# Mehran-Memon/fspann-query-system

Hardware: AMD Instinct MI355X
Metric: queries/sec @ recall@10, SIFT-1M-shaped synthetic data d=128 B=256 (higher is better)
Workload: dtype f64

## Files before the change

fspann-query-system_amd/csrc/route_lazy.hip.h:

```cpp
#pragma once
#include "route.hip.h"

namespace fspann {

constexpr uint64_t kLzEmpty = ~0ull;
constexpr int kLzThreads = 256;
constexpr int kLzEntriesMax = 1024;
constexpr int kLzCollMax = 256;
constexpr int lz_ht_size(int kEnt) { return 2 * kEnt; }
constexpr int lz_sort_max(int kEnt) { return kEnt - 128; }
constexpr size_t lz_order_bytes(int TP) {
    return static_cast<size_t>(TP + 2) * 8 + ((static_cast<size_t>(TP + 1) * 4 + 7) & ~size_t(7)) + static_cast<size_t>(TP) * 8 +
           ((static_cast<size_t>(TP) * 2 + 3) & ~size_t(3));
}
constexpr size_t lz_lds_bytes(int kEnt, int TD, int P) {
    const size_t tp = static_cast<size_t>(TD) * P, ord_gk = lz_order_bytes(TD * P), gk = static_cast<size_t>(lz_sort_max(kEnt)) * 4;
    return static_cast<size_t>(lz_ht_size(kEnt)) * 8 + tp * 16 + static_cast<size_t>(kEnt) * 4 + 4096 +
           (((ord_gk > gk ? ord_gk : gk) + 7) & ~size_t(7)) + static_cast<size_t>(TD) * 8 + static_cast<size_t>(kEnt) * 2 +
           static_cast<size_t>(lz_sort_max(kEnt)) * 2 * 2 + static_cast<size_t>(TD) * 4 +
           (kEnt != 512 ? static_cast<size_t>(TD) * 4 + tp * 4 : 0);
}
static_assert(lz_lds_bytes(512, 16, 5) == 20152 && lz_lds_bytes(512, 16, 5) + 256 <= 160 * 1024 / 8, "eight per CU at 16 x 5");
constexpr int lz_stage_u(int) { return 4; }
constexpr int lz_keep(int) { return 8; }

#ifdef FSPANN_DEBUG_STAMPS
__device__ __forceinline__ long long dbg_hw_where() {
    uint32_t hw, xcc;
    asm volatile("s_getreg_b32 %0, hwreg(HW_REG_HW_ID)" : "=s"(hw));
    asm volatile("s_getreg_b32 %0, hwreg(HW_REG_XCC_ID)" : "=s"(xcc));
    return (static_cast<long long>(xcc) << 32) | hw;
}
#endif

__device__ __forceinline__ int wave_cut1024(const int32_t* bins, int need, int lane, int* before) {
    const int4* b4 = reinterpret_cast<const int4*>(bins) + lane * 4;
    const int4 v0 = b4[0], v1 = b4[1], v2 = b4[2], v3 = b4[3];
    const int vals[16] = {v0.x, v0.y, v0.z, v0.w, v1.x, v1.y, v1.z, v1.w, v2.x, v2.y, v2.z, v2.w, v3.x, v3.y, v3.z, v3.w};
    int sum = 0;
#pragma unroll
    for (int i = 0; i < 16; i++) sum += vals[i];
    int incl = sum;
#pragma unroll
    for (int off = 1; off < 64; off <<= 1) {
        const int v = __shfl_up(incl, off);
        if (lane >= off) incl += v;
    }
    const int excl = incl - sum;
    const unsigned long long bm = __ballot((incl >= need) && (excl < need));
    if (bm == 0) {
        *before = __shfl(incl, 63) - __shfl(v3.w, 63);
        return 1023;
    }
    const int src = __ffsll(static_cast<long long>(bm)) - 1;
    int cum = excl, bb = 15;
    bool found = false;
#pragma unroll
    for (int i = 0; i < 16; i++) {
        if (!found) {
            if (cum + vals[i] >= need) { bb = i; found = true; }
            else cum += vals[i];
        }
    }
    *before = __shfl(cum, src);
    return __shfl(lane * 16 + bb, src);
}

template <int kThreads, int kEnt = kLzEntriesMax, bool kChk = true, int kTD = 0, int kP = 0, bool kList = false>
__device__ __forceinline__ void route_lazy_run(const RouteParams& prm, unsigned char* smem, const int64_t q_first, const int64_t q_stride, const int block_id) {
    int4* probe_in = prm.probe_g;
    int32_t* nprobe_in = prm.nprobe_g;
    int tid = threadIdx.x;
    constexpr int nthreads = kThreads;
    constexpr int nwv = kThreads / 64;
    int lane = tid & 63, wave = __builtin_amdgcn_readfirstlane(tid >> 6);
    const int TD = kTD > 0 ? kTD : prm.TD, P = kP > 0 ? kP : prm.P, S = (kTD > 0) ? 64 : prm.S;
    const int TP = TD * P;
    const int SP = (S + 63) >> 6;

    constexpr int kLzHtSize = lz_ht_size(kEnt), kLzEntries = kEnt, kLzSortMax = lz_sort_max(kEnt);
    constexpr int kLzStageU = lz_stage_u(kEnt), kLzKeep = lz_keep(kEnt);
    static_assert(kEnt == 512 || kEnt == 1024 || kEnt == 2048, "size classes");
    static_assert(!(kChk && kEnt == 512), "the 512-entry class has no registers for the check");
    size_t o = 0;
    uint64_t* ht = reinterpret_cast<uint64_t*>(smem + o);        o += static_cast<size_t>(kLzHtSize) * 8;
    int4* plist = reinterpret_cast<int4*>(smem + o);             o += static_cast<size_t>(TP) * 16;
    uint32_t* pre = reinterpret_cast<uint32_t*>(smem + o);       o += static_cast<size_t>(kEnt) * 4;
    int32_t* bins = reinterpret_cast<int32_t*>(smem + o);        o += 1024 * 4;
    const size_t o_ord = o;
    uint2* pkv = reinterpret_cast<uint2*>(smem + o);             o += (static_cast<size_t>(TP) + 2) * 8;
    int32_t* pcs = reinterpret_cast<int32_t*>(smem + o);         o += (static_cast<size_t>(TP) + 1) * 4;
    o = (o + 7) & ~size_t(7);
    int64_t* pbase = reinterpret_cast<int64_t*>(smem + o);       o += static_cast<size_t>(TP) * 8;
    uint16_t* ord = reinterpret_cast<uint16_t*>(smem + o);
    uint32_t* gk = reinterpret_cast<uint32_t*>(smem + o_ord);
    o = o_ord + ((max(lz_order_bytes(TP), static_cast<size_t>(kLzSortMax) * 4) + 7) & ~size_t(7));
    int64_t* ids_base = reinterpret_cast<int64_t*>(smem + o);    o += static_cast<size_t>(TD) * 8;
    uint16_t* ulist = reinterpret_cast<uint16_t*>(smem + o);     o += static_cast<size_t>(kLzEntries) * 2;
    uint16_t* rk = reinterpret_cast<uint16_t*>(smem + o);        o += static_cast<size_t>(kLzSortMax) * 2;
    uint16_t* lrank = reinterpret_cast<uint16_t*>(smem + o);     o += static_cast<size_t>(kLzSortMax) * 2;
    int32_t* nprobe_l = reinterpret_cast<int32_t*>(smem + o);    o += static_cast<size_t>(TD) * 4;
    int32_t* part0 = reinterpret_cast<int32_t*>(smem + o);       if (kEnt != 512) o += static_cast<size_t>(TD) * 4;
    int32_t* pglob = reinterpret_cast<int32_t*>(smem + o);
    int32_t* c_elem = bins;
    int32_t* c_lt = bins + kLzCollMax;
    int32_t* c_id = bins + 2 * kLzCollMax;
    int32_t* c_seq = bins + 3 * kLzCollMax;

    __shared__ int s_u, s_R, s_ncoll, s_bad, s_b, s_cnt, s_short, s_susp;
    constexpr uint32_t ht_mask = kLzHtSize - 1;
    constexpr int ht_shift = (kEnt == 2048) ? 32 - 12 : (kEnt == 1024) ? 32 - 11 : 32 - 10;
    unsigned long long lt_mask = 0;

    for (int i = tid; i < TD; i += nthreads) { ids_base[i] = prm.tables[i].ids_base; if (kChk) part0[i] = static_cast<int32_t>(prm.tables[i].part_base); }
    for (int i = tid; i < kLzHtSize; i += nthreads) ht[i] = kLzEmpty;
    if (kChk && prm.bin16) for (int i = tid; i < 1024; i += nthreads) bins[i] = 0;
    if (block_id == 0 && tid == 0) *prm.ovf_next = 0;
    __syncthreads();

    auto present = [&](int32_t id) -> bool {
        uint32_t slot = (static_cast<uint32_t>(id) * 2654435761u) >> ht_shift;
        const uint32_t stp = ((static_cast<uint32_t>(id) * 0x85EBCA6Bu) >> ht_shift) | 1u;
        for (int tries = 0; tries < kLzHtSize; tries++) {
            const uint64_t e = ht[slot];
            if (e == kLzEmpty) return false;
            if (static_cast<uint32_t>(e >> 32) == static_cast<uint32_t>(id)) return true;
            slot = (slot + stp) & ht_mask;
        }
        return false;
    };
    auto insert = [&](int32_t id, uint32_t low, uint32_t* slot_out) -> bool {
        const uint64_t mine = (static_cast<uint64_t>(static_cast<uint32_t>(id)) << 32) | low;
        uint32_t slot = (static_cast<uint32_t>(id) * 2654435761u) >> ht_shift;
        const uint32_t stp = ((static_cast<uint32_t>(id) * 0x85EBCA6Bu) >> ht_shift) | 1u;
        for (int tries = 0; tries < kLzHtSize; tries++) {
            const uint64_t old = atomicCAS(reinterpret_cast<unsigned long long*>(&ht[slot]), kLzEmpty, mine);
            if (old == kLzEmpty) { *slot_out = slot; return true; }
            if (static_cast<uint32_t>(old >> 32) == static_cast<uint32_t>(id)) {
                if (static_cast<uint32_t>(old) > low) atomicMin(reinterpret_cast<unsigned long long*>(&ht[slot]), mine);
                return false;
            }
            slot = (slot + stp) & ht_mask;
        }
        s_bad = 1;
        return false;
    };

#ifdef FSPANN_DEBUG_STAMPS
#define LZ_STAMP(i) do { if (prm.dbg && tid == 0 && qi == block_id) prm.dbg[block_id * 16 + (i)] = wall_clock64(); } while (0)
#else
#define LZ_STAMP(i) do { } while (0)
#endif
#ifdef FSPANN_LZ_STOP_AFTER
#define LZ_STOP(n) if (FSPANN_LZ_STOP_AFTER == (n) && prm.nq > 0) { __syncthreads(); if (tid == 0) prm.out_count[qi] = 0;               \
        const int used_ = min(s_u, kLzEntries); for (int i_ = tid; i_ < used_; i_ += nthreads) ht[ulist[i_]] = kLzEmpty; __syncthreads(); continue; }
#else
#define LZ_STOP(n)
#endif
#define LZ_FOR_TUPLES(RA, RB, BODY)                                                                                   \
    do {                                                                                                              \
        const int nit_ = ((RB) - (RA)) * SP;                                                                          \
        for (int it0_ = wave; it0_ < nit_; it0_ += nwv * kLzStageU) {                                                 \
            uint64_t entv_[kLzStageU];                                                                                \
            int scv_[kLzStageU];                                                                                      \
            _Pragma("unroll") for (int v_ = 0; v_ < kLzStageU; v_++) {                                                \
                const int it_ = it0_ + v_ * nwv;                                                                      \
                entv_[v_] = kLzEmpty; scv_[v_] = 0;                                                                   \
                if (it_ < nit_) {                                                                                     \
                    const int rr_ = (RA) + it_ / SP, pos_ = (it_ % SP) * 64 + lane;                                   \
                    const int pi_ = ord[rr_];                                                                         \
                    const int4 pr_ = plist[pi_];                                                                      \
                    scv_[v_] = pr_.y;                                                                                 \
                    if (pos_ < pr_.w) entv_[v_] = prm.ids_bk[pbase[pi_] + pos_];                                      \
                }                                                                                                     \
            }                                                                                                         \
            _Pragma("unroll") for (int v_ = 0; v_ < kLzStageU; v_++) {                                                \
                if (it0_ + v_ * nwv >= nit_) continue;                                                                \
                int32_t id = static_cast<int32_t>(entv_[v_] >> 32);                              \
                const uint32_t bf = static_cast<uint32_t>(entv_[v_]); (void)bf;                                       \
                const int sc = scv_[v_]; (void)sc;                                                                    \
                if (id >= 0 && prm.deleted_bits && ((prm.deleted_bits[id >> 5] >> (id & 31)) & 1u)) id = -1;  \
                BODY                                                                                                  \
            }                                                                                                         \
        }                                                                                                             \
    } while (0)
#define LZ_INSERT(COND, LOW)                                                                                          \
    do {                                                                                                              \
        bool created_ = false;                                                                                        \
        uint32_t slot_ = 0;                                                                                           \
        if (COND) created_ = insert(id, (LOW), &slot_);                                                               \
        const unsigned long long bm_ = __ballot(created_);                                                            \
        if (bm_) {                                                                                                    \
            int base_ = 0;                                                                                            \
            if (lane == 0) base_ = atomicAdd(&s_u, __popcll(bm_));                                                    \
            base_ = __shfl(base_, 0);                                                                                 \
            const int at_ = base_ + __popcll(bm_ & lt_mask);                                                          \
            if (created_ && at_ < kLzEntries) ulist[at_] = static_cast<uint16_t>(slot_);                              \
        }                                                                                                             \
    } while (0)

    const int64_t nq_eff = kList ? static_cast<int64_t>(*prm.qcount) : prm.nq;
    for (int64_t qs = q_first; qs < nq_eff; qs += q_stride) {
        const int64_t qi = kList ? static_cast<int64_t>(prm.qlist[qs]) : qs;
        LZ_STAMP(0);
        if (prm.probe_G > 0) {
            const int G = (kTD > 0) ? 16 : prm.probe_G, lgG = 31 - __clz(G), ngroups = nthreads >> lgG;
            const int grp_in_wave = lane >> lgG, gl = lane & (G - 1), grp = tid >> lgG;
            int32_t* w3 = reinterpret_cast<int32_t*>(pre) + grp * (2 * P - 1) * 3;
            for (int t0 = 0; t0 < TD; t0 += ngroups) {
                const int td = t0 + grp;
                const bool act = td < TD;
                const int tdc = act ? td : 0;
                const int Wc = (kTD > 0) ? 1 : prm.W;
#ifdef FSPANN_DEBUG_STAMPS
                long long* pst = (prm.dbg && tid == 0 && qi == block_id && t0 == 0) ? prm.dbg + (static_cast<long long>(gridDim.x) + block_id) * 16 : nullptr;
#else
                long long* pst = nullptr;
#endif
                const int np = route_probe_table<int4*, kP, (kTD > 0 ? 1 : 0)>(prm, act, prm.codes + (qi * TD + tdc) * Wc, prm.tables[tdc], G, gl, grp_in_wave,
                                                                             w3, plist + tdc * P, pst);
                if (act && gl == 0) nprobe_l[td] = np;
            }
            __syncthreads();
            for (int i = tid; i < TP; i += nthreads) {
                const int td = i / P, step = i - td * P;
                int4 e = make_int4(-1, 0x7FFF, 0, 0);
                if (step < nprobe_l[td]) e = plist[i];
                plist[i] = e;
                pbase[i] = ids_base[td] + e.z;
                if (kChk) pglob[i] = part0[td] + e.x;
                pkv[i] = make_uint2((static_cast<uint32_t>(e.y) << 16) | static_cast<uint32_t>(i), static_cast<uint32_t>(e.w));
            }
        } else {
            for (int i = tid; i < TP; i += nthreads) {
                const int td = i / P, step = i - td * P;
                int4 e = make_int4(-1, 0x7FFF, 0, 0);
                if (step < nprobe_in[qi * TD + td]) e = probe_in[qi * TP + i];
                plist[i] = e;
                pbase[i] = ids_base[td] + e.z;
                if (kChk) pglob[i] = part0[td] + e.x;
                pkv[i] = make_uint2((static_cast<uint32_t>(e.y) << 16) | static_cast<uint32_t>(i), static_cast<uint32_t>(e.w));
            }
        }
        if (tid == 0) {
            s_u = 0; s_R = TP; s_ncoll = 0; s_bad = 0; s_short = 0; s_susp = 0;
            if (TP & 1) pkv[TP] = make_uint2(0xFFFFFFFFu, 0u);
        }
        __syncthreads();
        LZ_STAMP(1);
        LZ_STOP(1)
        asm volatile("" : "+v"(tid));
        lane = tid & 63; wave = __builtin_amdgcn_readfirstlane(tid >> 6);
        lt_mask = (1ull << lane) - 1ull;
        constexpr int kChkU = 5;
        uint2 chk_v[kChkU];
        int chk_n[kChkU];
        const int chk_cps = prm.bin16_shift - 2;
        const int chk_items = (kChk && prm.bin16) ? (TP << chk_cps) : 0;
        const bool chk_once = chk_items <= nthreads * kChkU;
        auto chk_load = [&](const int it0) {
#pragma unroll
            for (int v = 0; v < kChkU; v++) {
                const int it = it0 + v * nthreads;
                chk_v[v] = make_uint2(0u, 0u); chk_n[v] = 0;
                if (it < chk_items) {
                    const int pi = it >> chk_cps, ch = it & ((1 << chk_cps) - 1);
                    const int4 pr = plist[pi];
                    const int rem = pr.w - ch * 4;
                    if (pr.x >= 0 && rem > 0) {
                        chk_v[v] = *reinterpret_cast<const uint2*>(prm.bin16 + (static_cast<int64_t>(pglob[pi]) << prm.bin16_shift) + ch * 4);
                        chk_n[v] = min(rem, 4);
                    }
                }
            }
        };
        auto chk_count = [&]() {
            bool sus = false;
#pragma unroll
            for (int v = 0; v < kChkU; v++) {
#pragma unroll
                for (int k = 0; k < 4; k++) {
                    if (k < chk_n[v]) {
                        const uint32_t b16 = ((k < 2 ? chk_v[v].x : chk_v[v].y) >> ((k & 1) * 16)) & 0xFFFFu;
                        const uint32_t sh = (b16 & 7u) * 4u;
                        const uint32_t old = atomicAdd(reinterpret_cast<uint32_t*>(bins) + ((b16 & 8191u) >> 3), 1u << sh);
                        sus = sus || (((old >> sh) & 15u) >= 8u);
                    }
                }
            }
            if (sus) s_susp = 1;
        };
        if (chk_items > 0 && chk_once) chk_load(tid);
        for (int i = tid; i < TP; i += nthreads) {
            const uint2 me = pkv[i];
            const uint32_t mk = me.x;
            int rank = 0, cum = 0;
            const uint4* kv4 = reinterpret_cast<const uint4*>(pkv);
#pragma unroll 4
            for (int j = 0; j < (TP + 1) / 2; j++) {
                const uint4 kv = kv4[j];
                const bool b0 = kv.x < mk, b1 = kv.z < mk;
                rank += b0 + b1;
                cum += (b0 ? kv.y : 0u) + (b1 ? kv.w : 0u);
            }
            ord[rank] = static_cast<uint16_t>(i);
            pcs[rank] = cum;
            if ((mk >> 16) == 0x7FFFu) atomicMin(&s_R, rank);
            if (rank == TP - 1) pcs[TP] = cum + static_cast<int>(me.y);
        }
        if (chk_items > 0) {
            if (chk_once) chk_count();
            else for (int it0 = tid; it0 < chk_items; it0 += nthreads * kChkU) { chk_load(it0); chk_count(); }
        }
        __syncthreads();
        LZ_STAMP(2);
        LZ_STOP(2)
        const int R = s_R;
        bool overflow = false;
        if (chk_items > 0 && s_susp) {
            uint32_t* mark = reinterpret_cast<uint32_t*>(ht);
            uint64_t* cl = ht + 128;
            uint64_t* cf = cl + 256;
            constexpr int kChkList = 256;
            static_assert(128 + 2 * 256 <= lz_ht_size(512), "the check's scratch fits the smallest hash table");
            for (int i = tid; i < 256; i += nthreads) mark[i] = 0u;
            for (int i = tid; i < 1024; i += nthreads) bins[i] = 0;
            __syncthreads();
            for (int it = tid; it < chk_items; it += nthreads) {
                const int pi = it >> chk_cps, ch = it & ((1 << chk_cps) - 1);
                const int4 pr = plist[pi];
                const int rem = pr.w - ch * 4;
                if (pr.x < 0 || rem <= 0) continue;
                const uint2 vv = *reinterpret_cast<const uint2*>(prm.bin16 + (static_cast<int64_t>(pglob[pi]) << prm.bin16_shift) + ch * 4);
                for (int k = 0; k < min(rem, 4); k++) {
                    const uint32_t b16 = ((k < 2 ? vv.x : vv.y) >> ((k & 1) * 16)) & 0xFFFFu, f = b16 & 8191u;
                    const uint32_t sh = (f & 7u) * 4u;
                    const uint32_t old = atomicAdd(reinterpret_cast<uint32_t*>(bins) + (f >> 3), 1u << sh);
                    if (((old >> sh) & 15u) >= 8u) atomicOr(&mark[f >> 5], 1u << (f & 31u));
                }
            }
            __syncthreads();
            for (int it = tid; it < chk_items; it += nthreads) {
                const int pi = it >> chk_cps, ch = it & ((1 << chk_cps) - 1);
                const int4 pr = plist[pi];
                const int rem = pr.w - ch * 4;
                if (pr.x < 0 || rem <= 0) continue;
                const uint2 vv = *reinterpret_cast<const uint2*>(prm.bin16 + (static_cast<int64_t>(pglob[pi]) << prm.bin16_shift) + ch * 4);
                for (int k = 0; k < min(rem, 4); k++) {
                    const uint32_t b16 = ((k < 2 ? vv.x : vv.y) >> ((k & 1) * 16)) & 0xFFFFu, f = b16 & 8191u;
                    if (!((mark[f >> 5] >> (f & 31u)) & 1u)) continue;
                    const int32_t id = prm.ids[pbase[pi] + ch * 4 + k];
                    if (prm.deleted_bits && ((prm.deleted_bits[id >> 5] >> (id & 31)) & 1u)) continue;
                    const int c = atomicAdd(&s_ncoll, 1);
                    if (c < kChkList) cl[c] = (static_cast<uint64_t>(b16) << 32) | static_cast<uint32_t>(id);
                }
            }
            __syncthreads();
            const int ncl = s_ncoll;
            if (ncl > kChkList) {
                overflow = true;
            } else {
                for (int i = tid; i < ncl; i += nthreads) {
                    const uint64_t me = cl[i];
                    bool first = true;
                    for (int j = 0; j < i; j++) first = first && (cl[j] != me);
                    cf[i] = first ? me : ~0ull;
                }
                __syncthreads();
                for (int i = tid; i < ncl; i += nthreads) {
                    const uint64_t me = cf[i];
                    if (me == ~0ull) continue;
                    int same = 0;
                    for (int j = 0; j < ncl; j++) same += (cf[j] != ~0ull) && ((cf[j] >> 32) == (me >> 32));
                    if (same >= 9) s_bad = 1;
                }
            }
            __syncthreads();
            if (s_bad) overflow = true;
            for (int i = tid; i < 128 + 2 * kChkList; i += nthreads) ht[i] = kLzEmpty;
            if (tid == 0) s_ncoll = 0;
            __syncthreads();
        }
        int r0 = 0, u = 0;
        int dbg_outer = 0, dbg_inner = 0, dbg_reload = 0, dbg_nitb = 0;
        (void)dbg_outer; (void)dbg_inner; (void)dbg_reload; (void)dbg_nitb;
        bool force_full = false;
        while (r0 < R && u < prm.limit && !overflow) {
            const int need = prm.limit - u;
            int r_fit = r0, r_nofit = R;
            for (int c0 = r0 + 1; c0 <= R; c0 += 64) {
                const int r = c0 + lane;
                const bool bnd = (r <= R) && (r == R || (pkv[ord[r]].x >> 16) != (pkv[ord[r - 1]].x >> 16));
                const unsigned long long bb = __ballot(bnd);
                const unsigned long long bf = __ballot(bnd && (pcs[r] - pcs[r0] <= need));
                if (bf) r_fit = c0 + 63 - __clzll(static_cast<long long>(bf));
                if (bb & ~bf) { r_nofit = c0 + __ffsll(static_cast<long long>(bb & ~bf)) - 1; break; }
            }
            const int rb0 = r_fit, rb1 = (r_fit < R) ? r_nofit : R;
            const int npB = rb1 - rb0;
            auto tuples_per_id = [](const int tuples, const int ids) -> int {
                return (tuples >= 8 * ids) ? 128 : (tuples >= 4 * ids) ? 64 : (tuples >= 3 * ids) ? 48 : (tuples >= 2 * ids) ? 32 : (2 * tuples >= 3 * ids) ? 24 : 16;
            };
            int boost = 16;
            if (r0 > 0 && u > 0) boost = min(64, tuples_per_id(pcs[r0], u));
            int L = 64;
            if (npB > 0 && SP == 1 && !force_full) {
                const int tuplesB = max(pcs[rb1] - pcs[rb0], 1);
                const int want = (2 * 64 * ((need * boost) >> 4)) / tuplesB + 8;
                L = (want <= 8) ? 8 : (want <= 16) ? 16 : (want <= 32) ? 32 : 64;
            }
            const int Lsh = 31 - __clz(L);
            const int G = 64 >> Lsh;
            const int nitB = (L == 64) ? npB * SP : (npB + G - 1) / G;
            const bool keep = (nitB > 0) && (nitB <= nwv * kLzKeep);
            dbg_outer++; dbg_reload += (nitB > 0 && !keep); dbg_nitb = max(dbg_nitb, nitB);
            int32_t idr[kLzKeep];
            uint32_t bfr[kLzKeep];
            if (keep) {
#pragma unroll
                for (int k = 0; k < kLzKeep; k++) {
                    const int it = wave + k * nwv;
                    idr[k] = -1; bfr[k] = 0;
                    if (it < nitB) {
                        int pidx, pos;
                        if (L == 64) { pidx = it / SP; pos = (it % SP) * 64 + lane; }
                        else { pidx = it * G + (lane >> Lsh); pos = lane & (L - 1); }
                        if (pidx < npB) {
                            const int pi = ord[rb0 + pidx];
                            const int4 pr = plist[pi];
                            if (pos < pr.w) {
                                const uint64_t ent = prm.ids_bk[pbase[pi] + pos];
                                idr[k] = static_cast<int32_t>(ent >> 32);
                                bfr[k] = static_cast<uint32_t>(ent) | ((L < 64 && pos == L - 1 && pr.w > L) ? 0x80000000u : 0u);
                            }
                        }
                    }
                }
            }
            for (int i = tid; i < 1024; i += nthreads) bins[i] = 0;
            if (r_fit > r0) {
                LZ_FOR_TUPLES(r0, r_fit, {
                    LZ_INSERT(id >= 0, (static_cast<uint32_t>(sc) << kBucketBits) | bf);
                });
            }
            __syncthreads();
            LZ_STAMP(8);
            u = s_u;
            if (s_bad) { overflow = true; break; }
            if (u >= prm.limit || rb0 >= R) {
                r0 = rb0;
                __syncthreads();
                continue;
            }
            const uint32_t sc_hi = (pkv[ord[rb0]].x >> 16) << kBucketBits;
            if (keep) {
#pragma unroll
                for (int k = 0; k < kLzKeep; k++) {
                    int32_t id = idr[k];
                    if (id >= 0 && prm.deleted_bits && ((prm.deleted_bits[id >> 5] >> (id & 31)) & 1u)) id = -1;
                    if (id >= 0) {
                        if (present(id)) id = -1;
                        else atomicAdd(&bins[(bfr[k] & 0xFFFFFu) >> (kBucketBits - 10)], 1);
                    }
                    idr[k] = id;
                }
            } else {
                LZ_FOR_TUPLES(rb0, rb1, {
                    if (id >= 0 && !present(id)) atomicAdd(&bins[bf >> (kBucketBits - 10)], 1);
                });
            }
            __syncthreads();
            LZ_STAMP(10);
            int lo = 0;
            bool redo_full = false;
            if (rb0 > 0 && u > 0) boost = min(64, tuples_per_id(pcs[rb0], u));
            while (true) {
                const int missing = prm.limit - u;
                const int ask = max(missing, min((missing * boost) >> 4, ((prm.lazy_cap - u) * 3) >> 2));
                if (wave == 0) {
                    int before = 0;
                    const int b = (lo == 0) ? wave_cut1024(bins, ask, lane, &before)
                                            : lo + wave_find_cut(bins + lo, 1024 - lo, ask, lane, &before);
                    if (lane == 0) { s_b = b; s_cnt = before + bins[b]; }
                }
                __syncthreads();
                LZ_STAMP(11);
                dbg_inner++;
                const int b = s_b;
                const int offered = s_cnt;
                if (u + offered > prm.lazy_cap) { overflow = true; break; }
                if (keep && L < 64) {
                    bool shortp = false;
#pragma unroll
                    for (int k = 0; k < kLzKeep; k++)
                        shortp = shortp || ((bfr[k] & 0x80000000u) && static_cast<int>((bfr[k] & 0xFFFFFu) >> (kBucketBits - 10)) <= b);
                    if (__any(shortp) && lane == 0) s_short = 1;
                    __syncthreads();
                    if (s_short) { redo_full = true; break; }
                }
                if (keep) {
                    int total = 0;
#pragma unroll
                    for (int k = 0; k < kLzKeep; k++) {
                        const int bin = static_cast<int>((bfr[k] & 0xFFFFFu) >> (kBucketBits - 10));
                        if (idr[k] >= 0 && bin >= lo && bin <= b) {
                            uint32_t slot = 0;
                            const bool c = insert(idr[k], sc_hi | (bfr[k] & 0xFFFFFu), &slot);
                            idr[k] = c ? -2 : -1;
                            if (c) bfr[k] = slot;
                        }
                        total += __popcll(__ballot(idr[k] == -2));
                    }
                    if (total) {
                        int base = 0;
                        if (lane == 0) base = atomicAdd(&s_u, total);
                        base = __shfl(base, 0);
#pragma unroll
                        for (int k = 0; k < kLzKeep; k++) {
                            const bool c = (idr[k] == -2);
                            const unsigned long long bm = __ballot(c);
                            const int at = base + __popcll(bm & lt_mask);
                            if (c && at < kLzEntries) ulist[at] = static_cast<uint16_t>(bfr[k]);
                            if (c) idr[k] = -1;
                            base += __popcll(bm);
                        }
                    }
                } else {
                    LZ_FOR_TUPLES(rb0, rb1, {
                        const int bin = static_cast<int>(bf >> (kBucketBits - 10));
                        LZ_INSERT(id >= 0 && bin >= lo && bin <= b, sc_hi | bf);
                    });
                }
                __syncthreads();
                LZ_STAMP(12);
                const int u_was = u;
                u = s_u;
                if (s_bad) { overflow = true; break; }
                if (u >= prm.limit || b >= 1023) break;
                boost = tuples_per_id(offered, max(u - u_was, 1));
                lo = b + 1;
                __syncthreads();
            }
            if (overflow) break;
            if (redo_full) {
                r0 = rb0;
                force_full = true;
                __syncthreads();
                if (tid == 0) s_short = 0;
                __syncthreads();
                continue;
            }
            force_full = false;
            r0 = rb1;
            __syncthreads();
        }
        LZ_STAMP(3);
        LZ_STOP(3)
        const int nsel = u;
        if (nsel > kLzSortMax) overflow = true;
        if (!overflow) {
            const int nout = min(nsel, prm.limit);
            const uint32_t smin = pkv[ord[0]].x >> 16;
            auto coarse = [&](const uint32_t key) -> uint32_t { return min((key - (smin << kBucketBits)) >> (kBucketBits - 6), 1023u); };
            for (int i = tid; i < kEnt; i += nthreads) pre[i] = (i < nsel) ? static_cast<uint32_t>(ht[ulist[i]]) : 0xFFFFFFFFu;
            for (int i = tid; i < kLzSortMax / 2; i += nthreads) reinterpret_cast<uint32_t*>(rk)[i] = 0u;
            for (int i = tid; i < 1024; i += nthreads) bins[i] = 0;
            __syncthreads();
            LZ_STAMP(4);
            for (int i = tid; i < nsel; i += nthreads) atomicAdd(&bins[coarse(pre[i])], 1);
            __syncthreads();
            if (wave == 0) {
                int4* b4 = reinterpret_cast<int4*>(bins) + lane * 4;
                int4 v[4] = {b4[0], b4[1], b4[2], b4[3]};
                int* vals = reinterpret_cast<int*>(v);
                int sum = 0;
#pragma unroll
                for (int i = 0; i < 16; i++) { const int t = vals[i]; vals[i] = sum; sum += t; }
                int incl = sum;
#pragma unroll
                for (int off = 1; off < 64; off <<= 1) {
                    const int t = __shfl_up(incl, off);
                    if (lane >= off) incl += t;
                }
                const int excl = incl - sum;
#pragma unroll
                for (int i = 0; i < 16; i++) vals[i] += excl;
                b4[0] = v[0]; b4[1] = v[1]; b4[2] = v[2]; b4[3] = v[3];
            }
            __syncthreads();
            for (int i = tid; i < nsel; i += nthreads) {
                const uint32_t my = pre[i];
                gk[atomicAdd(&bins[coarse(my)], 1)] = my;
            }
            __syncthreads();
            for (int i = tid; i < nsel; i += nthreads) {
                const uint32_t my = pre[i];
                const uint32_t c = coarse(my);
                const int g1 = bins[c], g0 = c ? bins[c - 1] : 0;
                int lt = g0;
                for (int j = g0; j < g1; j++) lt += gk[j] < my;
                atomicAdd(reinterpret_cast<uint32_t*>(rk) + (lt >> 1), 1u << ((lt & 1) * 16));
                lrank[i] = static_cast<uint16_t>(lt);
            }
            __syncthreads();
            for (int i = tid; i < nsel; i += nthreads) {
                const int lt = lrank[i];
                if (rk[lt] != 1) {
                    if (rk[lt] >= 9) s_bad = 1;
                    const int c = atomicAdd(&s_ncoll, 1);
                    if (c < kLzCollMax) { c_elem[c] = i; c_lt[c] = lt; c_id[c] = static_cast<int32_t>(ht[ulist[i]] >> 32); c_seq[c] = 0x7FFFFFFF; }
                }
            }
            __syncthreads();
            LZ_STAMP(5);
            LZ_STOP(5)
            const int ncoll = s_ncoll;
#ifdef FSPANN_DEBUG_STAMPS
            if (tid == 0 && prm.dbg && qi == block_id) { prm.dbg[block_id * 16 + 13] = ncoll; prm.dbg[block_id * 16 + 15] = nsel; prm.dbg[block_id * 16 + 14] = dbg_outer | (dbg_inner << 8) | (dbg_reload << 16) | (static_cast<long long>(dbg_nitb) << 24); }
#endif
            if (ncoll > kLzCollMax || s_bad) {
                overflow = true;
            } else {
                if (ncoll > 0) {
                    const int npair = ncoll * TD;
                    for (int t0 = tid; t0 < npair; t0 += nthreads * 4) {
                        int32_t idxv[4];
#pragma unroll
                        for (int v = 0; v < 4; v++) {
                            const int t = t0 + v * nthreads;
                            idxv[v] = (t < npair) ? prm.inv[static_cast<int64_t>(t % TD) * prm.n_ids + c_id[t / TD]] : -1;
                        }
#pragma unroll
                        for (int v = 0; v < 4; v++) {
                            const int t = t0 + v * nthreads;
                            const int32_t idx = idxv[v];
                            if (idx < 0) continue;
                            const int c = t / TD, td = t - c * TD;
                            for (int step = 0; step < P; step++) {
                                const int4 e = plist[td * P + step];
                                if (e.x >= 0 && idx >= e.z && idx < e.z + e.w) { atomicMin(&c_seq[c], (td * P + step) * S + (idx - e.z)); break; }
                            }
                        }
                    }
                    for (int c = tid; c < ncoll; c += nthreads) c_elem[c] = static_cast<int32_t>(pre[c_elem[c]]);
                    __syncthreads();
                    for (int c = tid; c < ncoll; c += nthreads) {
                        const int32_t my = c_elem[c];
                        const int myseq = c_seq[c];
                        int rank = c_lt[c];
#pragma unroll 4
                        for (int c2 = 0; c2 < ncoll; c2++) rank += (c_elem[c2] == my) && (c_seq[c2] < myseq);
                        if (rank < nout) {
                            prm.out_ids[qi * prm.out_cap + rank] = c_id[c];
                            if (prm.out_score) prm.out_score[qi * prm.out_cap + rank] = static_cast<int32_t>(static_cast<uint32_t>(my) >> kBucketBits);
                        }
                    }
                }
                for (int i = tid; i < nsel; i += nthreads) {
                    const int lt = lrank[i];
                    if (lt < nout && rk[lt] == 1) {
                        const uint64_t e = ht[ulist[i]];
                        prm.out_ids[qi * prm.out_cap + lt] = static_cast<int32_t>(e >> 32);
                        if (prm.out_score) prm.out_score[qi * prm.out_cap + lt] = static_cast<int32_t>(static_cast<uint32_t>(e) >> kBucketBits);
                    }
                }
            }
            if (!overflow && tid == 0) prm.out_count[qi] = nout;
        }
        if (overflow) {
            if (prm.probe_G > 0) {
                for (int i = tid; i < TP; i += nthreads) probe_in[qi * TP + i] = plist[i];
                for (int i = tid; i < TD; i += nthreads) nprobe_in[qi * TD + i] = nprobe_l[i];
            }
            if (tid == 0) {
                prm.out_count[qi] = kRoutePending;
                prm.ovf_list[atomicAdd(prm.ovf_count, 1)] = static_cast<int32_t>(qi);
            }
        }
        if (qs + q_stride >= nq_eff) {
            LZ_STAMP(6);
            LZ_STAMP(7);
            break;
        }
        __syncthreads();
        LZ_STAMP(6);
        const int used = min(s_u, kLzEntries);
        for (int i = tid; i < used; i += nthreads) ht[ulist[i]] = kLzEmpty;
        if (kChk && prm.bin16) for (int i = tid; i < 1024; i += nthreads) bins[i] = 0;
        __syncthreads();
        LZ_STAMP(7);
    }
#undef LZ_STOP
#undef LZ_STAMP
#undef LZ_FOR_TUPLES
#undef LZ_INSERT
}

template <int kThreads, int kEnt, bool kChk, int kTD = 0, int kP = 0>
__global__ __launch_bounds__(kThreads, (kEnt <= 512 ? (kTD > 0 ? 8 : 6) : (kEnt <= 1024 ? 4 : 2))) void route_select_lazy_kernel(RouteParams prm) {
    extern __shared__ __align__(16) unsigned char smem[];
#ifdef FSPANN_DEBUG_STAMPS
    if (prm.dbg && threadIdx.x == 0) prm.dbg[blockIdx.x * 16 + 9] = dbg_hw_where();
#endif
    route_lazy_run<kThreads, kEnt, kChk, kTD, kP>(prm, smem, static_cast<int64_t>(blockIdx.x), static_cast<int64_t>(gridDim.x), static_cast<int>(blockIdx.x));
}

template <int kThreads, int kEnt, bool kChk>
__global__ __launch_bounds__(kThreads, (kEnt <= 512 ? 6 : (kEnt <= 1024 ? 4 : 2))) void route_select_lazy_list_kernel(RouteParams prm) {
    extern __shared__ __align__(16) unsigned char smem[];
    if (static_cast<int64_t>(blockIdx.x) >= static_cast<int64_t>(*prm.qcount)) {
        if (blockIdx.x == 0 && threadIdx.x == 0) *prm.ovf_next = 0;
        return;
    }
    route_lazy_run<kThreads, kEnt, kChk, 0, 0, true>(prm, smem, static_cast<int64_t>(blockIdx.x), static_cast<int64_t>(gridDim.x), static_cast<int>(blockIdx.x));
}

}
```

Baseline: 26.95 million.

## Batch hash-table probes and inserts across tuples in lockstep rounds

Replaces the per-tuple serial hash probe and insert loops with batched round-based routines. Each lane advances several ids at once, which interleaves LDS accesses and removes divergent loops. Tuple loading is made branch-free with clamped indices, deleted-bit lookups are batched, and shared scalars are pinned uniform with readfirstlane to favour scalar registers. The trade-off is higher register pressure from the per-lane state arrays and some extra masked work per round.

Result: slower. 26.53 million (-1.6%).

```diff
diff --git a/fspann-query-system_amd/csrc/route_lazy.hip.h b/fspann-query-system_amd/csrc/route_lazy.hip.h
--- a/fspann-query-system_amd/csrc/route_lazy.hip.h
+++ b/fspann-query-system_amd/csrc/route_lazy.hip.h
@@ -66,6 +66,94 @@
     return __shfl(lane * 16 + bb, src);
 }
 
+__device__ __forceinline__ int64_t lz_uniform64(const int64_t v) {
+    const uint32_t lo = __builtin_amdgcn_readfirstlane(static_cast<uint32_t>(v)), hi = __builtin_amdgcn_readfirstlane(static_cast<uint32_t>(static_cast<uint64_t>(v) >> 32));
+    return static_cast<int64_t>((static_cast<uint64_t>(hi) << 32) | lo);
+}
+
+template <int kHtSize>
+__device__ __forceinline__ uint32_t lz_hash_state(const int32_t id) {
+    constexpr int sh = (kHtSize == 4096) ? 32 - 12 : (kHtSize == 2048) ? 32 - 11 : 32 - 10;
+    static_assert(kHtSize == 4096 || kHtSize == 2048 || kHtSize == 1024, "32 - log2(hash slots)");
+    const uint32_t slot = (static_cast<uint32_t>(id) * 2654435761u) >> sh;
+    const uint32_t stp = ((static_cast<uint32_t>(id) * 0x85EBCA6Bu) >> sh) | 1u;
+    return slot | (stp << 16);
+}
+template <int kHtSize>
+__device__ __forceinline__ uint32_t lz_hash_next(const uint32_t st) { return (st & 0xFFFF0000u) | ((st + (st >> 16)) & static_cast<uint32_t>(kHtSize - 1)); }
+
+template <int kHtSize, int N>
+__device__ __forceinline__ uint32_t lz_present_rounds(const uint64_t* ht, const int32_t* id, uint32_t pend) {
+    uint32_t st[N];
+#pragma unroll
+    for (int k = 0; k < N; k++) st[k] = lz_hash_state<kHtSize>(id[k]);
+    uint32_t found = 0;
+    for (int tries = 0; tries < kHtSize && __ballot(pend != 0u) != 0ull; tries++) {
+#pragma unroll
+        for (int k = 0; k < N; k++) {
+            const uint32_t bit = 1u << k;
+            if (__ballot((pend & bit) != 0u) != 0ull) {
+                const uint32_t hi = static_cast<uint32_t>(ht[st[k] & 0xFFFFu] >> 32);
+                const bool hit = hi == static_cast<uint32_t>(id[k]);
+                const bool on = !hit && hi != 0xFFFFFFFFu;
+                found |= hit ? (pend & bit) : 0u;
+                pend &= on ? ~0u : ~bit;
+                st[k] = on ? lz_hash_next<kHtSize>(st[k]) : st[k];
+            }
+        }
+    }
+    return found;
+}
+
+template <int kHtSize, int N>
+__device__ __forceinline__ uint32_t lz_insert_rounds(uint64_t* ht, const int32_t* id, const uint32_t* low, uint32_t pend, uint32_t* st, int* s_bad) {
+#pragma unroll
+    for (int k = 0; k < N; k++) st[k] = lz_hash_state<kHtSize>(id[k]);
+    uint32_t created = 0;
+    for (int tries = 0; tries < kHtSize && __ballot(pend != 0u) != 0ull; tries++) {
+#pragma unroll
+        for (int k = 0; k < N; k++) {
+            const uint32_t bit = 1u << k;
+            if (__ballot((pend & bit) != 0u) != 0ull) {
+                const bool p = (pend & bit) != 0u;
+                const uint32_t lw = low[k];
+                const uint64_t mine = (static_cast<uint64_t>(static_cast<uint32_t>(id[k])) << 32) | lw;
+                unsigned long long* const at = reinterpret_cast<unsigned long long*>(&ht[st[k] & 0xFFFFu]);
+                uint64_t old = 0;
+                if (p) old = atomicCAS(at, kLzEmpty, mine);
+                const bool won = p && old == kLzEmpty;
+                const bool same = p && static_cast<uint32_t>(old >> 32) == static_cast<uint32_t>(id[k]);
+                if (same && static_cast<uint32_t>(old) > lw) atomicMin(at, mine);
+                created |= won ? bit : 0u;
+                pend &= (won || same) ? ~bit : ~0u;
+                st[k] = (p && !won && !same) ? lz_hash_next<kHtSize>(st[k]) : st[k];
+            }
+        }
+    }
+    if (__ballot(pend != 0u) != 0ull) { if (pend != 0u) *s_bad = 1; }
+    return created;
+}
+
+template <int kEnt, int N>
+__device__ __forceinline__ void lz_append_created(const uint32_t created, const uint32_t* st, int* s_u, uint16_t* ulist, const int lane) {
+    int total = 0;
+#pragma unroll
+    for (int k = 0; k < N; k++) total += __popcll(__ballot((created >> k) & 1u));
+    if (total) {
+        int base = 0;
+        if (lane == 0) base = atomicAdd(s_u, total);
+        base = __builtin_amdgcn_readfirstlane(base);
+#pragma unroll
+        for (int k = 0; k < N; k++) {
+            const bool c = (created >> k) & 1u;
+            const unsigned long long bm = __ballot(c);
+            const int at = base + static_cast<int>(__builtin_amdgcn_mbcnt_hi(static_cast<uint32_t>(bm >> 32), __builtin_amdgcn_mbcnt_lo(static_cast<uint32_t>(bm), 0u)));
+            if (c && at < kEnt) ulist[at] = static_cast<uint16_t>(st[k] & 0xFFFFu);
+            base += __popcll(bm);
+        }
+    }
+}
+
 template <int kThreads, int kEnt = kLzEntriesMax, bool kChk = true, int kTD = 0, int kP = 0, bool kList = false>
 __device__ __forceinline__ void route_lazy_run(const RouteParams& prm, unsigned char* smem, const int64_t q_first, const int64_t q_stride, const int block_id) {
     int4* probe_in = prm.probe_g;
@@ -80,6 +168,7 @@
 
     constexpr int kLzHtSize = lz_ht_size(kEnt), kLzEntries = kEnt, kLzSortMax = lz_sort_max(kEnt);
     constexpr int kLzStageU = lz_stage_u(kEnt), kLzKeep = lz_keep(kEnt);
+    constexpr int kLzRoundN = kLzKeep;
     static_assert(kEnt == 512 || kEnt == 1024 || kEnt == 2048, "size classes");
     static_assert(!(kChk && kEnt == 512), "the 512-entry class has no registers for the check");
     size_t o = 0;
@@ -108,43 +197,12 @@
     int32_t* c_seq = bins + 3 * kLzCollMax;
 
     __shared__ int s_u, s_R, s_ncoll, s_bad, s_b, s_cnt, s_short, s_susp;
-    constexpr uint32_t ht_mask = kLzHtSize - 1;
-    constexpr int ht_shift = (kEnt == 2048) ? 32 - 12 : (kEnt == 1024) ? 32 - 11 : 32 - 10;
-    unsigned long long lt_mask = 0;
 
     for (int i = tid; i < TD; i += nthreads) { ids_base[i] = prm.tables[i].ids_base; if (kChk) part0[i] = static_cast<int32_t>(prm.tables[i].part_base); }
     for (int i = tid; i < kLzHtSize; i += nthreads) ht[i] = kLzEmpty;
     if (kChk && prm.bin16) for (int i = tid; i < 1024; i += nthreads) bins[i] = 0;
     if (block_id == 0 && tid == 0) *prm.ovf_next = 0;
     __syncthreads();
-
-    auto present = [&](int32_t id) -> bool {
-        uint32_t slot = (static_cast<uint32_t>(id) * 2654435761u) >> ht_shift;
-        const uint32_t stp = ((static_cast<uint32_t>(id) * 0x85EBCA6Bu) >> ht_shift) | 1u;
-        for (int tries = 0; tries < kLzHtSize; tries++) {
-            const uint64_t e = ht[slot];
-            if (e == kLzEmpty) return false;
-            if (static_cast<uint32_t>(e >> 32) == static_cast<uint32_t>(id)) return true;
-            slot = (slot + stp) & ht_mask;
-        }
-        return false;
-    };
-    auto insert = [&](int32_t id, uint32_t low, uint32_t* slot_out) -> bool {
-        const uint64_t mine = (static_cast<uint64_t>(static_cast<uint32_t>(id)) << 32) | low;
-        uint32_t slot = (static_cast<uint32_t>(id) * 2654435761u) >> ht_shift;
-        const uint32_t stp = ((static_cast<uint32_t>(id) * 0x85EBCA6Bu) >> ht_shift) | 1u;
-        for (int tries = 0; tries < kLzHtSize; tries++) {
-            const uint64_t old = atomicCAS(reinterpret_cast<unsigned long long*>(&ht[slot]), kLzEmpty, mine);
-            if (old == kLzEmpty) { *slot_out = slot; return true; }
-            if (static_cast<uint32_t>(old >> 32) == static_cast<uint32_t>(id)) {
-                if (static_cast<uint32_t>(old) > low) atomicMin(reinterpret_cast<unsigned long long*>(&ht[slot]), mine);
-                return false;
-            }
-            slot = (slot + stp) & ht_mask;
-        }
-        s_bad = 1;
-        return false;
-    };
 
 #ifdef FSPANN_DEBUG_STAMPS
 #define LZ_STAMP(i) do { if (prm.dbg && tid == 0 && qi == block_id) prm.dbg[block_id * 16 + (i)] = wall_clock64(); } while (0)
@@ -157,47 +215,33 @@
 #else
 #define LZ_STOP(n)
 #endif
-#define LZ_FOR_TUPLES(RA, RB, BODY)                                                                                   \
+#define LZ_FOR_TRIPS(RA, RB, ...)                                                                                 \
     do {                                                                                                              \
         const int nit_ = ((RB) - (RA)) * SP;                                                                          \
         for (int it0_ = wave; it0_ < nit_; it0_ += nwv * kLzStageU) {                                                 \
-            uint64_t entv_[kLzStageU];                                                                                \
-            int scv_[kLzStageU];                                                                                      \
+            int32_t idv[kLzStageU];                                                                                   \
+            uint32_t lowv[kLzStageU];                                                                                 \
             _Pragma("unroll") for (int v_ = 0; v_ < kLzStageU; v_++) {                                                \
-                const int it_ = it0_ + v_ * nwv;                                                                      \
-                entv_[v_] = kLzEmpty; scv_[v_] = 0;                                                                   \
-                if (it_ < nit_) {                                                                                     \
-                    const int rr_ = (RA) + it_ / SP, pos_ = (it_ % SP) * 64 + lane;                                   \
-                    const int pi_ = ord[rr_];                                                                         \
-                    const int4 pr_ = plist[pi_];                                                                      \
-                    scv_[v_] = pr_.y;                                                                                 \
-                    if (pos_ < pr_.w) entv_[v_] = prm.ids_bk[pbase[pi_] + pos_];                                      \
-                }                                                                                                     \
+                const int it_ = it0_ + v_ * nwv, itc_ = min(it_, nit_ - 1);                                           \
+                const int rr_ = (RA) + itc_ / SP, pos_ = (itc_ % SP) * 64 + lane;                                     \
+                 \
+                const int pi_ = __builtin_amdgcn_readfirstlane(ord[rr_]);                                             \
+                const int sc_ = __builtin_amdgcn_readfirstlane(plist[pi_].y), w_ = __builtin_amdgcn_readfirstlane(plist[pi_].w); \
+                const uint64_t* row_ = prm.ids_bk + lz_uniform64(pbase[pi_]);                                         \
+                const uint64_t ent_ = row_[static_cast<uint32_t>(min(pos_, max(w_, 1) - 1))];                         \
+                const bool live_ = (it_ < nit_) && (pos_ < w_);                                                       \
+                idv[v_] = live_ ? static_cast<int32_t>(ent_ >> 32) : -1;                                              \
+                lowv[v_] = (static_cast<uint32_t>(sc_) << kBucketBits) | static_cast<uint32_t>(ent_);                 \
             }                                                                                                         \
-            _Pragma("unroll") for (int v_ = 0; v_ < kLzStageU; v_++) {                                                \
-                if (it0_ + v_ * nwv >= nit_) continue;                                                                \
-                int32_t id = static_cast<int32_t>(entv_[v_] >> 32);                              \
-                const uint32_t bf = static_cast<uint32_t>(entv_[v_]); (void)bf;                                       \
-                const int sc = scv_[v_]; (void)sc;                                                                    \
-                if (id >= 0 && prm.deleted_bits && ((prm.deleted_bits[id >> 5] >> (id & 31)) & 1u)) id = -1;  \
-                BODY                                                                                                  \
+            if (prm.deleted_bits) {                                                                       \
+                uint32_t dw_[kLzStageU];                                                                              \
+                _Pragma("unroll") for (int v_ = 0; v_ < kLzStageU; v_++) dw_[v_] = prm.deleted_bits[static_cast<uint32_t>(max(idv[v_], 0)) >> 5]; \
+                _Pragma("unroll") for (int v_ = 0; v_ < kLzStageU; v_++) idv[v_] = ((dw_[v_] >> (idv[v_] & 31)) & 1u) ? -1 : idv[v_]; \
             }                                                                                                         \
+            __VA_ARGS__                                                                                               \
         }                                                                                                             \
     } while (0)
-#define LZ_INSERT(COND, LOW)                                                                                          \
-    do {                                                                                                              \
-        bool created_ = false;                                                                                        \
-        uint32_t slot_ = 0;                                                                                           \
-        if (COND) created_ = insert(id, (LOW), &slot_);                                                               \
-        const unsigned long long bm_ = __ballot(created_);                                                            \
-        if (bm_) {                                                                                                    \
-            int base_ = 0;                                                                                            \
-            if (lane == 0) base_ = atomicAdd(&s_u, __popcll(bm_));                                                    \
-            base_ = __shfl(base_, 0);                                                                                 \
-            const int at_ = base_ + __popcll(bm_ & lt_mask);                                                          \
-            if (created_ && at_ < kLzEntries) ulist[at_] = static_cast<uint16_t>(slot_);                              \
-        }                                                                                                             \
-    } while (0)
+#define LZ_BITS(N, WHAT) ([&]() -> uint32_t { uint32_t m_ = 0; _Pragma("unroll") for (int v = 0; v < (N); v++) m_ |= (WHAT) ? (1u << v) : 0u; return m_; }())
 
     const int64_t nq_eff = kList ? static_cast<int64_t>(*prm.qcount) : prm.nq;
     for (int64_t qs = q_first; qs < nq_eff; qs += q_stride) {
@@ -251,7 +295,6 @@
         LZ_STOP(1)
         asm volatile("" : "+v"(tid));
         lane = tid & 63; wave = __builtin_amdgcn_readfirstlane(tid >> 6);
-        lt_mask = (1ull << lane) - 1ull;
         constexpr int kChkU = 5;
         uint2 chk_v[kChkU];
         int chk_n[kChkU];
@@ -315,7 +358,7 @@
         __syncthreads();
         LZ_STAMP(2);
         LZ_STOP(2)
-        const int R = s_R;
+        const int R = __builtin_amdgcn_readfirstlane(s_R);
         bool overflow = false;
         if (chk_items > 0 && s_susp) {
             uint32_t* mark = reinterpret_cast<uint32_t*>(ht);
@@ -402,10 +445,10 @@
                 return (tuples >= 8 * ids) ? 128 : (tuples >= 4 * ids) ? 64 : (tuples >= 3 * ids) ? 48 : (tuples >= 2 * ids) ? 32 : (2 * tuples >= 3 * ids) ? 24 : 16;
             };
             int boost = 16;
-            if (r0 > 0 && u > 0) boost = min(64, tuples_per_id(pcs[r0], u));
+            if (r0 > 0 && u > 0) boost = min(64, tuples_per_id(__builtin_amdgcn_readfirstlane(pcs[r0]), u));
             int L = 64;
             if (npB > 0 && SP == 1 && !force_full) {
-                const int tuplesB = max(pcs[rb1] - pcs[rb0], 1);
+                const int tuplesB = max(__builtin_amdgcn_readfirstlane(pcs[rb1] - pcs[rb0]), 1);
                 const int want = (2 * 64 * ((need * boost) >> 4)) / tuplesB + 8;
                 L = (want <= 8) ? 8 : (want <= 16) ? 16 : (want <= 32) ? 32 : 64;
             }
@@ -414,13 +457,15 @@
             const int nitB = (L == 64) ? npB * SP : (npB + G - 1) / G;
             const bool keep = (nitB > 0) && (nitB <= nwv * kLzKeep);
             dbg_outer++; dbg_reload += (nitB > 0 && !keep); dbg_nitb = max(dbg_nitb, nitB);
+            const uint32_t sc_hi = (rb0 < R) ? __builtin_amdgcn_readfirstlane((pkv[ord[rb0]].x >> 16) << kBucketBits) : 0u;
             int32_t idr[kLzKeep];
-            uint32_t bfr[kLzKeep];
+            uint32_t lwr[kLzKeep];
+            uint32_t shortm = 0;
             if (keep) {
 #pragma unroll
                 for (int k = 0; k < kLzKeep; k++) {
                     const int it = wave + k * nwv;
-                    idr[k] = -1; bfr[k] = 0;
+                    idr[k] = -1; lwr[k] = 0;
                     if (it < nitB) {
                         int pidx, pos;
                         if (L == 64) { pidx = it / SP; pos = (it % SP) * 64 + lane; }
@@ -431,7 +476,8 @@
                             if (pos < pr.w) {
                                 const uint64_t ent = prm.ids_bk[pbase[pi] + pos];
                                 idr[k] = static_cast<int32_t>(ent >> 32);
-                                bfr[k] = static_cast<uint32_t>(ent) | ((L < 64 && pos == L - 1 && pr.w > L) ? 0x80000000u : 0u);
+                                lwr[k] = sc_hi | static_cast<uint32_t>(ent);
+                                shortm |= (L < 64 && pos == L - 1 && pr.w > L) ? (1u << k) : 0u;
                             }
                         }
                     }
@@ -439,41 +485,50 @@
             }
             for (int i = tid; i < 1024; i += nthreads) bins[i] = 0;
             if (r_fit > r0) {
-                LZ_FOR_TUPLES(r0, r_fit, {
-                    LZ_INSERT(id >= 0, (static_cast<uint32_t>(sc) << kBucketBits) | bf);
+                LZ_FOR_TRIPS(r0, r_fit, {
+                    uint32_t st[kLzStageU];
+                    const uint32_t created = lz_insert_rounds<kLzHtSize, kLzStageU>(ht, idv, lowv, LZ_BITS(kLzStageU, idv[v] >= 0), st, &s_bad);
+                    lz_append_created<kLzEntries, kLzStageU>(created, st, &s_u, ulist, lane);
                 });
             }
             __syncthreads();
             LZ_STAMP(8);
-            u = s_u;
-            if (s_bad) { overflow = true; break; }
+            u = __builtin_amdgcn_readfirstlane(s_u);
+            if (__builtin_amdgcn_readfirstlane(s_bad)) { overflow = true; break; }
             if (u >= prm.limit || rb0 >= R) {
                 r0 = rb0;
                 __syncthreads();
                 continue;
             }
-            const uint32_t sc_hi = (pkv[ord[rb0]].x >> 16) << kBucketBits;
             if (keep) {
+                if (prm.deleted_bits) {
+                    uint32_t dw[kLzKeep];
+#pragma unroll
+                    for (int k = 0; k < kLzKeep; k++) dw[k] = prm.deleted_bits[static_cast<uint32_t>(max(idr[k], 0)) >> 5];
+#pragma unroll
+                    for (int k = 0; k < kLzKeep; k++) idr[k] = ((dw[k] >> (idr[k] & 31)) & 1u) ? -1 : idr[k];
+                }
+                uint32_t have = 0;
+#pragma unroll
+                for (int h = 0; h < kLzKeep; h += kLzRoundN)
+                    have |= lz_present_rounds<kLzHtSize, kLzRoundN>(ht, idr + h, LZ_BITS(kLzRoundN, idr[h + v] >= 0)) << h;
 #pragma unroll
                 for (int k = 0; k < kLzKeep; k++) {
-                    int32_t id = idr[k];
-                    if (id >= 0 && prm.deleted_bits && ((prm.deleted_bits[id >> 5] >> (id & 31)) & 1u)) id = -1;
-                    if (id >= 0) {
-                        if (present(id)) id = -1;
-                        else atomicAdd(&bins[(bfr[k] & 0xFFFFFu) >> (kBucketBits - 10)], 1);
-                    }
-                    idr[k] = id;
+                    if ((have >> k) & 1u) idr[k] = -1;
+                    if (idr[k] >= 0) atomicAdd(&bins[(lwr[k] & 0xFFFFFu) >> (kBucketBits - 10)], 1);
                 }
             } else {
-                LZ_FOR_TUPLES(rb0, rb1, {
-                    if (id >= 0 && !present(id)) atomicAdd(&bins[bf >> (kBucketBits - 10)], 1);
+                LZ_FOR_TRIPS(rb0, rb1, {
+                    const uint32_t have = lz_present_rounds<kLzHtSize, kLzStageU>(ht, idv, LZ_BITS(kLzStageU, idv[v] >= 0));
+                    _Pragma("unroll") for (int v = 0; v < kLzStageU; v++)
+                        if (idv[v] >= 0 && !((have >> v) & 1u)) atomicAdd(&bins[(lowv[v] & 0xFFFFFu) >> (kBucketBits - 10)], 1);
                 });
             }
             __syncthreads();
             LZ_STAMP(10);
             int lo = 0;
             bool redo_full = false;
-            if (rb0 > 0 && u > 0) boost = min(64, tuples_per_id(pcs[rb0], u));
+            if (rb0 > 0 && u > 0) boost = min(64, tuples_per_id(__builtin_amdgcn_readfirstlane(pcs[rb0]), u));
             while (true) {
                 const int missing = prm.limit - u;
                 const int ask = max(missing, min((missing * boost) >> 4, ((prm.lazy_cap - u) * 3) >> 2));
@@ -486,56 +541,49 @@
                 __syncthreads();
                 LZ_STAMP(11);
                 dbg_inner++;
-                const int b = s_b;
-                const int offered = s_cnt;
+                const int b = __builtin_amdgcn_readfirstlane(s_b);
+                const int offered = __builtin_amdgcn_readfirstlane(s_cnt);
                 if (u + offered > prm.lazy_cap) { overflow = true; break; }
                 if (keep && L < 64) {
                     bool shortp = false;
 #pragma unroll
                     for (int k = 0; k < kLzKeep; k++)
-                        shortp = shortp || ((bfr[k] & 0x80000000u) && static_cast<int>((bfr[k] & 0xFFFFFu) >> (kBucketBits - 10)) <= b);
+                        shortp = shortp || (((shortm >> k) & 1u) && static_cast<int>((lwr[k] & 0xFFFFFu) >> (kBucketBits - 10)) <= b);
                     if (__any(shortp) && lane == 0) s_short = 1;
                     __syncthreads();
-                    if (s_short) { redo_full = true; break; }
+                    if (__builtin_amdgcn_readfirstlane(s_short)) { redo_full = true; break; }
                 }
                 if (keep) {
-                    int total = 0;
-#pragma unroll
-                    for (int k = 0; k < kLzKeep; k++) {
-                        const int bin = static_cast<int>((bfr[k] & 0xFFFFFu) >> (kBucketBits - 10));
-                        if (idr[k] >= 0 && bin >= lo && bin <= b) {
-                            uint32_t slot = 0;
-                            const bool c = insert(idr[k], sc_hi | (bfr[k] & 0xFFFFFu), &slot);
-                            idr[k] = c ? -2 : -1;
-                            if (c) bfr[k] = slot;
-                        }
-                        total += __popcll(__ballot(idr[k] == -2));
-                    }
-                    if (total) {
-                        int base = 0;
-                        if (lane == 0) base = atomicAdd(&s_u, total);
-                        base = __shfl(base, 0);
-#pragma unroll
-                        for (int k = 0; k < kLzKeep; k++) {
-                            const bool c = (idr[k] == -2);
-                            const unsigned long long bm = __ballot(c);
-                            const int at = base + __popcll(bm & lt_mask);
-                            if (c && at < kLzEntries) ulist[at] = static_cast<uint16_t>(bfr[k]);
-                            if (c) idr[k] = -1;
-                            base += __popcll(bm);
+#pragma unroll
+                    for (int h = 0; h < kLzKeep; h += kLzRoundN) {
+                        const uint32_t want = LZ_BITS(kLzRoundN, idr[h + v] >= 0 && static_cast<int>((lwr[h + v] & 0xFFFFFu) >> (kBucketBits - 10)) >= lo &&
+                                                                     static_cast<int>((lwr[h + v] & 0xFFFFFu) >> (kBucketBits - 10)) <= b);
+                        uint32_t st[kLzRoundN];
+                        const uint32_t created = lz_insert_rounds<kLzHtSize, kLzRoundN>(ht, idr + h, lwr + h, want, st, &s_bad);
+#pragma unroll
+                        for (int k = 0; k < kLzRoundN; k++) {
+                            const bool c = (created >> k) & 1u;
+                            idr[h + k] = c ? -2 : ((want >> k) & 1u) ? -1 : idr[h + k];
+                            lwr[h + k] = c ? st[k] : lwr[h + k];
                         }
                     }
+                    lz_append_created<kLzEntries, kLzKeep>(LZ_BITS(kLzKeep, idr[v] == -2), lwr, &s_u, ulist, lane);
+#pragma unroll
+                    for (int k = 0; k < kLzKeep; k++) idr[k] = (idr[k] == -2) ? -1 : idr[k];
                 } else {
-                    LZ_FOR_TUPLES(rb0, rb1, {
-                        const int bin = static_cast<int>(bf >> (kBucketBits - 10));
-                        LZ_INSERT(id >= 0 && bin >= lo && bin <= b, sc_hi | bf);
+                    LZ_FOR_TRIPS(rb0, rb1, {
+                        const uint32_t want = LZ_BITS(kLzStageU, idv[v] >= 0 && static_cast<int>((lowv[v] & 0xFFFFFu) >> (kBucketBits - 10)) >= lo &&
+                                                                     static_cast<int>((lowv[v] & 0xFFFFFu) >> (kBucketBits - 10)) <= b);
+                        uint32_t st[kLzStageU];
+                        const uint32_t created = lz_insert_rounds<kLzHtSize, kLzStageU>(ht, idv, lowv, want, st, &s_bad);
+                        lz_append_created<kLzEntries, kLzStageU>(created, st, &s_u, ulist, lane);
                     });
                 }
                 __syncthreads();
                 LZ_STAMP(12);
                 const int u_was = u;
-                u = s_u;
-                if (s_bad) { overflow = true; break; }
+                u = __builtin_amdgcn_readfirstlane(s_u);
+                if (__builtin_amdgcn_readfirstlane(s_bad)) { overflow = true; break; }
                 if (u >= prm.limit || b >= 1023) break;
                 boost = tuples_per_id(offered, max(u - u_was, 1));
                 lo = b + 1;
@@ -685,15 +733,17 @@
         __syncthreads();
         LZ_STAMP(6);
         const int used = min(s_u, kLzEntries);
-        for (int i = tid; i < used; i += nthreads) ht[ulist[i]] = kLzEmpty;
+        uint64_t empty = kLzEmpty;
+        asm volatile("" : "+v"(empty));
+        for (int i = tid; i < used; i += nthreads) ht[ulist[i]] = empty;
         if (kChk && prm.bin16) for (int i = tid; i < 1024; i += nthreads) bins[i] = 0;
         __syncthreads();
         LZ_STAMP(7);
     }
 #undef LZ_STOP
 #undef LZ_STAMP
-#undef LZ_FOR_TUPLES
-#undef LZ_INSERT
+#undef LZ_FOR_TRIPS
+#undef LZ_BITS
 }
 
 template <int kThreads, int kEnt, bool kChk, int kTD = 0, int kP = 0>
```
